# taraak/pita

Measured on AMD Instinct MI355X. Metric: walker-steps/sec (batch x T) LJ13 @ 65k walkers/GPU, higher is better.
Workload: dtype f32

## Files before the change

pita_amd/csrc/egnn_common.h:

```cpp
#pragma once
#include <cstdlib>

#include "common.h"

namespace pita {

typedef float f32x16 __attribute__((ext_vector_type(16)));
typedef float f32x4 __attribute__((ext_vector_type(4)));

constexpr int EH = 32;
constexpr int PBS = 36;
constexpr int MAT_F = 1024;
enum { M_WA = 0, M_WB, M_W2, M_WC1, M_WN1A, M_WN1B, M_WN2,
       M_WAT, M_WBT, M_W2T, M_WC1T, M_WN1AT, M_WN1BT, M_WN2T, M_COUNT };
enum { V_WRE = 0 , V_B1 = 2, V_B2, V_WATT, V_BC1, V_WC2, V_BN1,
       V_BN2, V_WRF , V_WEF , V_COUNT };
constexpr int VEC_EMB_F = 96;
constexpr int VEC_LAYER_F = V_COUNT * EH + 4;


__device__ __forceinline__ void wave_lds_fence() {
  asm volatile("s_waitcnt lgkmcnt(0)" ::: "memory");
}

// ... 82 lines not shown
      acc = __builtin_amdgcn_mfma_f32_32x32x16_bf16(as_bf16x8(w[0][st]), as_bf16x8(x[1][st]), acc, 0, 0, 0);
      acc = __builtin_amdgcn_mfma_f32_32x32x16_bf16(as_bf16x8(w[0][st]), as_bf16x8(x[0][st]), acc, 0, 0, 0);
    }
    return acc;
  }
  __device__ __forceinline__ f32x16 mul(const f32x16& in, f32x16 acc) const {
    u32x4 x[3][2];
    split(in, x);
    return mul_split(x, acc);
  }
};

constexpr float F16_SX = 1.0f, F16_SW = 16.0f;
constexpr bool F16_NODE_LAYERS = true;
constexpr float F16_UNSCALE = 1.0f / (F16_SX * F16_SW);
constexpr float DIV_ST = 32.0f;
constexpr float DIV_SV = 2048.0f;
constexpr int VEC_DIV_F = 4 * EH;
constexpr int MAT_WH = 1024;
typedef _Float16 f16x8 __attribute__((ext_vector_type(8)));
typedef _Float16 f16x2 __attribute__((ext_vector_type(2)));
__device__ __forceinline__ f16x8 as_f16x8(u32x4 v) { return __builtin_bit_cast(f16x8, v); }
__device__ __forceinline__ float f16_rem_lo(unsigned pk, float x) {
  float r;
  asm("v_fma_mix_f32 %0, %1, -1.0, %2 op_sel:[0,0,0] op_sel_hi:[1,0,0]" : "=v"(r) : "v"(pk), "v"(x));
  return r;
}
__device__ __forceinline__ float f16_rem_hi(unsigned pk, float x) {
  float r;
  asm("v_fma_mix_f32 %0, %1, -1.0, %2 op_sel:[1,0,0] op_sel_hi:[1,0,0]" : "=v"(r) : "v"(pk), "v"(x));
  return r;
}

template <>
struct WFrag<2> {
  u32x4 w[2][2];
  __device__ __forceinline__ void load(const float* __restrict__, const unsigned* __restrict__ m16, int mat, int lane) {
    const u32x4* p = reinterpret_cast<const u32x4*>(m16 + (size_t)mat * MAT_WH) + lane;
#pragma unroll
    for (int pc = 0; pc < 2; ++pc)
#pragma unroll
      for (int st = 0; st < 2; ++st) w[pc][st] = p[(pc * 2 + st) * 64];
  }
  static __device__ __forceinline__ void split(const f32x16& in, u32x4 (&x)[2][2]) {
    typedef float f32x2_t __attribute__((ext_vector_type(2)));
#pragma unroll
    for (int st = 0; st < 2; ++st)
#pragma unroll
      for (int q = 0; q < 4; ++q) {
        const float a = in[8 * st + 2 * q], b = in[8 * st + 2 * q + 1];
        const unsigned p1 = __builtin_bit_cast(unsigned, __builtin_convertvector(f32x2_t{a, b}, f16x2));
        const float ra = f16_rem_lo(p1, a), rb = f16_rem_hi(p1, b);
        x[0][st][q] = p1;
        x[1][st][q] = __builtin_bit_cast(unsigned, __builtin_convertvector(f32x2_t{ra, rb}, f16x2));
      }
  }
  __device__ __forceinline__ f32x16 mul_split(const u32x4 (&x)[2][2], f32x16 acc) const {
#pragma unroll
    for (int st = 0; st < 2; ++st) {
      acc = __builtin_amdgcn_mfma_f32_32x32x16_f16(as_f16x8(w[1][st]), as_f16x8(x[0][st]), acc, 0, 0, 0);
      acc = __builtin_amdgcn_mfma_f32_32x32x16_f16(as_f16x8(w[0][st]), as_f16x8(x[1][st]), acc, 0, 0, 0);
      acc = __builtin_amdgcn_mfma_f32_32x32x16_f16(as_f16x8(w[0][st]), as_f16x8(x[0][st]), acc, 0, 0, 0);
    }
    return acc;
  }
  __device__ __forceinline__ f32x16 mul(const f32x16& in, f32x16 acc) const {
    u32x4 x[2][2];
    split(in, x);
    return mul_split(x, acc);
  }
};

typedef float f32x2 __attribute__((ext_vector_type(2)));
constexpr float SILU_PRESCALE = -1.44269504088896341f;
__device__ __forceinline__ f32x2 silu2(f32x2 v) {
  f32x2 e;
  e.x = __builtin_amdgcn_exp2f(v.x);
  e.y = __builtin_amdgcn_exp2f(v.y);
  const f32x2 d = e + 1.0f;
  f32x2 r;
  r.x = __builtin_amdgcn_rcpf(d.x);
  r.y = __builtin_amdgcn_rcpf(d.y);
  return v * r;
}
__device__ __forceinline__ void silu16(f32x16& m) {
  f32x2 e[8];
#pragma unroll
  for (int q = 0; q < 8; ++q) {
    e[q].x = __builtin_amdgcn_exp2f(m[2 * q]);
    e[q].y = __builtin_amdgcn_exp2f(m[2 * q + 1]);
  }
#pragma unroll
  for (int q = 0; q < 8; ++q) e[q] = e[q] + 1.0f;
#pragma unroll
  for (int q = 0; q < 8; ++q) {
    e[q].x = __builtin_amdgcn_rcpf(e[q].x);
    e[q].y = __builtin_amdgcn_rcpf(e[q].y);
  }
#pragma unroll
  for (int q = 0; q < 8; ++q) {
    const f32x2 y = f32x2{m[2 * q], m[2 * q + 1]} * e[q];
    m[2 * q] = y.x;
    m[2 * q + 1] = y.y;
  }
}
__device__ __forceinline__ f32x2 silu2_scaled(f32x2 v) {
  f32x2 e;
  e.x = __builtin_amdgcn_exp2f(v.x);
  e.y = __builtin_amdgcn_exp2f(v.y);
  const f32x2 c = {1.0f / F16_SX, 1.0f / F16_SX};
  const f32x2 d = __builtin_elementwise_fma(e, c, c);
  f32x2 r;
  r.x = __builtin_amdgcn_rcpf(d.x);
  r.y = __builtin_amdgcn_rcpf(d.y);
  return v * r;
}
#ifndef PITA_SILU_BATCH
#define PITA_SILU_BATCH 8
#endif
template <bool UNSCALE>
__device__ __forceinline__ void silu16_staged(f32x16& m) {
  constexpr int Q = PITA_SILU_BATCH;
  const f32x2 c = {1.0f / F16_SX, 1.0f / F16_SX};
#pragma unroll
  for (int q0 = 0; q0 < 8; q0 += Q) {
    f32x2 v[Q], e[Q];
#pragma unroll
    for (int q = 0; q < Q; ++q) {
      v[q] = f32x2{m[2 * (q0 + q)], m[2 * (q0 + q) + 1]};
      if (UNSCALE) v[q] = v[q] * F16_UNSCALE;
    }
#pragma unroll
    for (int q = 0; q < Q; ++q) {
      e[q].x = __builtin_amdgcn_exp2f(v[q].x);
      e[q].y = __builtin_amdgcn_exp2f(v[q].y);
    }
#pragma unroll
    for (int q = 0; q < Q; ++q) e[q] = __builtin_elementwise_fma(e[q], c, c);
#pragma unroll
    for (int q = 0; q < Q; ++q) {
      e[q].x = __builtin_amdgcn_rcpf(e[q].x);
      e[q].y = __builtin_amdgcn_rcpf(e[q].y);
    }
#pragma unroll
    for (int q = 0; q < Q; ++q) {
      const f32x2 y = v[q] * e[q];
      m[2 * (q0 + q)] = y.x;
      m[2 * (q0 + q) + 1] = y.y;
    }
  }
}
__device__ __forceinline__ void silu16_out(f32x16& m) { silu16_staged<false>(m); }
__device__ __forceinline__ void silu16_acc(f32x16& m) { silu16_staged<true>(m); }

__device__ __forceinline__ float dot16(const f32x16& w, const f32x16& m) {
  f32x2 acc = {0.f, 0.f};
#pragma unroll
  for (int q = 0; q < 8; ++q)
    acc = __builtin_elementwise_fma(f32x2{w[2 * q], w[2 * q + 1]}, f32x2{m[2 * q], m[2 * q + 1]}, acc);
  return acc.x + acc.y;
}

__device__ __forceinline__ float xhalf_sum(float v) {
  const unsigned u = __float_as_uint(v);
  const auto r = __builtin_amdgcn_permlane32_swap(u, u, false, false);
  return __uint_as_float(r[0]) + __uint_as_float(r[1]);
}

__device__ __forceinline__ void frag_to_agpr(WFrag<2>& f) {
#pragma unroll
  for (int pc = 0; pc < 2; ++pc)
#pragma unroll
    for (int st = 0; st < 2; ++st) asm volatile("" : "+a"(f.w[pc][st]));
}
__device__ __forceinline__ void frag_to_agpr(WFrag<1>& f) {
#pragma unroll
  for (int pc = 0; pc < 3; ++pc)
#pragma unroll
    for (int st = 0; st < 2; ++st) asm volatile("" : "+a"(f.w[pc][st]));
}

__device__ __forceinline__ float tanh_select(float v) {
  const float a = fabsf(v);
  const float v2 = v * v;
  float p = 62.0f / 2835.0f;
  p = fmaf(p, v2, -17.0f / 315.0f);
  p = fmaf(p, v2, 2.0f / 15.0f);
  p = fmaf(p, v2, -1.0f / 3.0f);
  p = fmaf(p, v2, 1.0f);
  float small = v * p;
  const float e = __builtin_amdgcn_exp2f(2.88539008177792681f * a);
  float big = copysignf(1.0f - 2.0f * __builtin_amdgcn_rcpf(1.0f + e), v);
  asm volatile("" : "+v"(small), "+v"(big));
  return a < 0.25f ? small : big;
}

}

struct PitaDeviceGuard {
  int prev = -1;
  bool switched = false;
  explicit PitaDeviceGuard(int device) {
    if (device >= 0 && hipGetDevice(&prev) == hipSuccess && prev != device) switched = hipSetDevice(device) == hipSuccess;
  }
  ~PitaDeviceGuard() {
    if (switched) (void)hipSetDevice(prev);
  }
  PitaDeviceGuard(const PitaDeviceGuard&) = delete;
  PitaDeviceGuard& operator=(const PitaDeviceGuard&) = delete;
};

struct pita_egnn {
  pita_egnn_config cfg;
  unsigned* d_mats16 = nullptr;
  unsigned* d_mats16h = nullptr;
  float* d_mats = nullptr;
  float* d_vecs = nullptr;
  float* d_vecs_h = nullptr;
  float* d_vecs_div = nullptr;
  int* d_vjp_mark = nullptr;
  size_t vjp_mark_bytes = 0;
  const void* shape = nullptr;
  const void* shape_small = nullptr;
  int n_cu = 256;
  int device = -1;
  float* d_ws = nullptr;
  size_t ws_bytes = 0;
  float* d_divcache = nullptr;
  size_t divcache_bytes = 0;
  int* d_mark = nullptr;
  size_t mark_bytes = 0;
  int div_seq = 0;
  void* d_bk = nullptr;
  size_t bk_bytes = 0;
};
```

pita_amd/csrc/egnn_kernel.hip:

```cpp
#include "egnn_common.h"

namespace pita {

struct EgnnParams {
  const unsigned* mats16;
  const unsigned* mats16h;
  const float* mats;
  const float* vecs;
  int n_layers, in_nf, attention, tanh_on, feature_layout;
  float coord_scale;
  int mode;
  long long B;
  const float* x_in;
  const float* t;
  const float* beta;
  float* out;
  float* x;
  const float* step_tab;
  int n_steps;
  const float* noise;
  unsigned long long seed, walker_offset;
  long long step0;
  int remove_mean;
  float* drift_out;
  double* stats_out;
  int repair;
  const float* x_backup;
  int* bad_from;
};

#ifndef PITA_EGNN_RECOMPUTE_COLS
#define PITA_EGNN_RECOMPUTE_COLS 1
#endif

template <int N, int DIM, int G, int WAVES>
struct EgnnCfg {
  static constexpr int NCOL = G * N;
  static constexpr int NT = (NCOL + 31) / 32;
  static constexpr int NCOLP = NT * 32;
  static constexpr int PB_F = NCOLP * PBS;
  static constexpr int POS_F = NCOLP * DIM;
  static constexpr int WAVE_F = PB_F + 4 * POS_F;
  static __host__ __device__ constexpr int vec_f(int L) { return ((VEC_EMB_F + L * VEC_LAYER_F) + 3) & ~3; }
  static __host__ __device__ constexpr size_t lds_bytes(int L) {
    return sizeof(float) * (size_t)(vec_f(L) + WAVES * WAVE_F);
  }
};

template <int N, int DIM, int G, int WAVES, int PREC, bool SAMPLER, int OCC = 2>
__global__ void __launch_bounds__(WAVES * 64, OCC) egnn_kernel(EgnnParams p) {
  const int mode = SAMPLER ? 3 : p.mode;
  using C = EgnnCfg<N, DIM, G, WAVES>;
  constexpr int NT = C::NT;
  extern __shared__ __attribute__((aligned(16))) float lds[];

  const int L = p.n_layers;
  const int vec_f = C::vec_f(L);
  for (int i = threadIdx.x; i < VEC_EMB_F + L * VEC_LAYER_F; i += WAVES * 64) lds[i] = p.vecs[i];
  __syncthreads();

  const int wave = threadIdx.x >> 6;
  const int lane = threadIdx.x & 63;
  const int cl = lane & 31;
  const int hh = lane >> 5;
  float* PB = lds + vec_f + wave * C::WAVE_F;
  float* posbuf0 = PB + C::PB_F;
  float* posbuf1 = posbuf0 + C::POS_F;
  float* pos0 = posbuf1 + C::POS_F;
  float* xbuf = pos0 + C::POS_F;
  const float* vemb = lds;

  const long long total_waves = (long long)gridDim.x * WAVES;
  const long long quota = (p.B + total_waves - 1) / total_waves;
  const long long wbeg = ((long long)blockIdx.x * WAVES + wave) * quota;
  const long long wend = (wbeg + quota < p.B) ? wbeg + quota : p.B;
  for (long long walker0 = wbeg; walker0 < wend; walker0 += G) {
    const int nwalk = (int)((wend - walker0) < G ? (wend - walker0) : G);
    const int ncol = nwalk * N;
    const int ntile = (ncol + 31) >> 5;
    int col[NT], nodei[NT];
    bool valid[NT];
    long long wid[NT];
    float xcur[NT][DIM];
#pragma unroll
    for (int T = 0; T < NT; ++T) {
      col[T] = T * 32 + cl;
      int w = col[T] / N;
      nodei[T] = col[T] - w * N;
      wid[T] = walker0 + w;
      valid[T] = (col[T] < ncol);
      if (!valid[T]) wid[T] = p.B - 1;
      const float* src = (mode == 3 ? p.x : p.x_in);
#pragma unroll
      for (int k = 0; k < DIM; ++k) xcur[T][k] = valid[T] ? src[(walker0 * N + col[T]) * DIM + k] : 0.0f;
    }
    int bad_from[NT];
#pragma unroll
    for (int T = 0; T < NT; ++T) bad_from[T] = 0x7fffffff;
    bool mine[NT];
#pragma unroll
    for (int T = 0; T < NT; ++T) mine[T] = valid[T];
    if (PREC != 2 && p.repair) {
      bool bad = false;
      float* flag = PB;
#pragma unroll
      for (int T = 0; T < NT; ++T) {
        bool b = false;
#pragma unroll
        for (int k = 0; k < DIM; ++k) {
          const float v = (mode == 3) ? xcur[T][k] : (valid[T] ? p.out[(walker0 * N + col[T]) * DIM + k] : 0.0f);
          b = b || !__builtin_isfinite(v);
        }
        if (hh == 0) flag[col[T]] = b ? 1.0f : 0.0f;
        bad = bad || b;
      }
      if (!__any(bad)) continue;
      wave_lds_fence();
#pragma unroll
      for (int T = 0; T < NT; ++T) {
        const int cb = (col[T] < ncol) ? col[T] - nodei[T] : 0;
        float any = 0.f;
        for (int q = 0; q < N; ++q) any += flag[cb + q];
        mine[T] = valid[T] && any != 0.f;
      }
      wave_lds_fence();
      if (mode == 3) {
#pragma unroll
        for (int T = 0; T < NT; ++T) {
#pragma unroll
          for (int k = 0; k < DIM; ++k)
            xcur[T][k] = valid[T] ? p.x_backup[(walker0 * N + col[T]) * DIM + k] : 0.0f;
          if (p.stats_out && p.bad_from && valid[T]) bad_from[T] = p.bad_from[walker0 * N + col[T]];
        }
      }
    }

#pragma unroll
    for (int T = 0; T < NT; ++T)
#pragma unroll
      for (int k = 0; k < DIM; ++k)
        if (hh == 0) xbuf[col[T] * DIM + k] = xcur[T][k];
    wave_lds_fence();

    const int nsteps = (mode == 3) ? p.n_steps : 1;
    for (int step = 0; step < nsteps; ++step) {
#if PITA_EGNN_RECOMPUTE_COLS
      int col[NT], nodei[NT];
      bool valid[NT];
      long long wid[NT];
      {
        int cl_o = cl;
        asm volatile("" : "+v"(cl_o));
#pragma unroll
        for (int T = 0; T < NT; ++T) {
          col[T] = T * 32 + cl_o;
          const int w = col[T] / N;
          nodei[T] = col[T] - w * N;
          wid[T] = walker0 + w;
          valid[T] = (col[T] < ncol);
          if (!valid[T]) wid[T] = p.B - 1;
        }
      }
#endif
      float c_s[NT], c_in[NT], c_out[NT], tfeat[NT], hval[NT], bfeat[NT];
      float g2 = 0.f, gamma = 0.f, dt = 0.f, noise_scale = 0.f, sqrt_dt = 0.f;
      if (mode == 3) {
        const float* st = p.step_tab + (size_t)step * PITA_STEP_STRIDE;
        auto uni = [&](int i) {
          return __builtin_bit_cast(float, __builtin_amdgcn_readfirstlane(__builtin_bit_cast(int, st[i])));
        };
        const float u_cs = uni(PITA_ST_CS), u_cin = uni(PITA_ST_CIN), u_cout = uni(PITA_ST_COUT),
                    u_cn = uni(PITA_ST_CNOISE), u_h = uni(PITA_ST_H), u_b = uni(PITA_ST_BETA);
#pragma unroll
        for (int T = 0; T < NT; ++T) {
          c_s[T] = u_cs; c_in[T] = u_cin; c_out[T] = u_cout;
          tfeat[T] = u_cn; hval[T] = u_h; bfeat[T] = u_b;
        }
        g2 = uni(PITA_ST_G2); gamma = uni(PITA_ST_GAMMA); dt = uni(PITA_ST_DT);
        noise_scale = uni(PITA_ST_NOISE_SCALE); sqrt_dt = uni(PITA_ST_SQRT_DT);
      } else {
#pragma unroll
        for (int T = 0; T < NT; ++T) {
          float tv = p.t[wid[T]];
          bfeat[T] = p.beta ? p.beta[wid[T]] : 0.0f;
          if (mode == 0) {
            c_s[T] = 0.f; c_in[T] = 1.f; c_out[T] = 1.f; tfeat[T] = tv; hval[T] = 1.f;
          } else {
            hval[T] = tv;
            c_s[T] = 1.0f / (1.0f + tv);
            c_in[T] = 1.0f / sqrtf(1.0f + tv);
            c_out[T] = sqrtf(tv) * c_in[T];
            tfeat[T] = 0.125f * logf(tv);
          }
        }
      }

      f32x16 hfeat[NT];
#pragma unroll
      for (int T = 0; T < NT; ++T) {
#pragma unroll
        for (int k = 0; k < DIM; ++k) {
          const float xc = xbuf[col[T] * DIM + k];
          const float ps = (mode == 0) ? xc : c_in[T] * xc;
          if (hh == 0) {
            pos0[col[T] * DIM + k] = ps;
            posbuf0[col[T] * DIM + k] = ps;
          }
        }
        float a0, a1;
        if (p.in_nf == 1) {
          a0 = tfeat[T]; a1 = 0.f;
        } else if (p.feature_layout == 0) {
          a0 = (2 * nodei[T] < N) ? tfeat[T] : bfeat[T];
          a1 = (2 * nodei[T] + 1 < N) ? tfeat[T] : bfeat[T];
        } else {
          a0 = tfeat[T]; a1 = bfeat[T];
        }
        f32x16 w0 = lds_vec16(vemb + hh * 16), w1 = lds_vec16(vemb + 32 + hh * 16), eb = lds_vec16(vemb + 64 + hh * 16);
#pragma unroll
        for (int r = 0; r < 16; ++r) hfeat[T][r] = fmaf(w0[r], a0, fmaf(w1[r], a1, eb[r]));
      }
      wave_lds_fence();

      float* poscur = posbuf0;
      float* posnext = posbuf1;
      for (int l = 0; l < L; ++l) {
        const float* mats = p.mats + (size_t)l * M_COUNT * MAT_F;
        const unsigned* mats16 = p.mats16 + (size_t)l * M_COUNT * MAT_W;
        const unsigned* mats16h = p.mats16h + (size_t)l * M_COUNT * MAT_WH;
        constexpr int NPREC = (PREC == 2 && !F16_NODE_LAYERS) ? 1 : PREC;
        constexpr bool NODE16 = (PREC == 2 && F16_NODE_LAYERS);
        const unsigned* matsn = NODE16 ? mats16h : mats16;
        const float* vl = lds + VEC_EMB_F + l * VEC_LAYER_F + hh * 16;
        const bool last = (l == L - 1);
        const float aggw = last ? 0.0f : (PREC == 2 ? 1.0f / F16_SX : 1.0f);
        {
          WFrag<NPREC> wb;
          wb.load(mats, matsn, M_WB, lane);
#pragma unroll
          for (int T = 0; T < NT; ++T) {
            if (T >= ntile) continue;
            f32x16 z = {0};
            f32x16 pb = wb.mul(hfeat[T], z);
            if (NODE16) pb *= F16_UNSCALE;
            f32x4* dst = reinterpret_cast<f32x4*>(PB + col[T] * PBS + hh * 16);
            dst[0] = f32x4{pb[0], pb[1], pb[2], pb[3]};
            dst[1] = f32x4{pb[4], pb[5], pb[6], pb[7]};
            dst[2] = f32x4{pb[8], pb[9], pb[10], pb[11]};
            dst[3] = f32x4{pb[12], pb[13], pb[14], pb[15]};
          }
        }
        wave_lds_fence();

        WFrag<PREC> w2f, wc1f;
        w2f.load(mats, PREC == 2 ? mats16h : mats16, M_W2, lane);
        wc1f.load(mats, PREC == 2 ? mats16h : mats16, M_WC1, lane);
        const float a_re = lds[VEC_EMB_F + l * VEC_LAYER_F + V_WRE * EH + lane];
        const float b_att = lds[VEC_EMB_F + l * VEC_LAYER_F + V_COUNT * EH];

#pragma unroll
        for (int T = 0; T < NT; ++T) {
          if (T >= ntile) continue;
          f32x16 Ai;
          {
            WFrag<NPREC> wa;
            wa.load(mats, matsn, M_WA, lane);
            Ai = wa.mul(hfeat[T], lds_vec16(vl + V_B1 * EH));
            if (NODE16) Ai *= F16_UNSCALE;
          }
          f32x16 agg = {0};
          float xacc[DIM], pown[DIM], p0own[DIM];
#pragma unroll
          for (int k = 0; k < DIM; ++k) {
            xacc[k] = 0.f;
            pown[k] = poscur[col[T] * DIM + k];
            p0own[k] = pos0[col[T] * DIM + k];
          }
          const int cbase = col[T] - nodei[T];

          for (int dd = 1; dd < N; ++dd) {
            asm volatile("" ::: "memory");
            int j = nodei[T] + dd;
            j = (j >= N) ? j - N : j;
            const int cj = (col[T] < ncol) ? cbase + j : col[T];
            float df[DIM], radial = 0.f, ea = 0.f;
#pragma unroll
            for (int k = 0; k < DIM; ++k) {
              df[k] = pown[k] - poscur[cj * DIM + k];
              radial = fmaf(df[k], df[k], radial);
              const float e0 = p0own[k] - pos0[cj * DIM + k];
              ea = fmaf(e0, e0, ea);
            }
            f32x16 m = Ai + lds_vec16(PB + cj * PBS + hh * 16);
            m = __builtin_amdgcn_mfma_f32_32x32x2f32(a_re, hh ? ea : radial, m, 0, 0, 0);
            __builtin_amdgcn_s_setprio(0);
            if (PREC == 2) silu16_out(m); else silu16(m);
            __builtin_amdgcn_s_setprio(1);
            m = w2f.mul(m, lds_vec16(vl + V_B2 * EH));
            __builtin_amdgcn_s_setprio(0);
            if (PREC == 2) silu16_acc(m); else silu16(m);
            __builtin_amdgcn_s_setprio(1);
            if (p.attention) {
              const float att = fast_sigmoid(xhalf_sum(dot16(lds_vec16(vl + V_WATT * EH), m)) + b_att);
              m *= att;
            }
#pragma unroll
            for (int r = 0; r < 16; ++r) agg[r] = fmaf(m[r], aggw, agg[r]);
            f32x16 c1 = wc1f.mul(m, lds_vec16(vl + V_BC1 * EH));
            __builtin_amdgcn_s_setprio(0);
            if (PREC == 2) silu16_acc(c1); else silu16(c1);
            __builtin_amdgcn_s_setprio(1);
            float cs = xhalf_sum(dot16(lds_vec16(vl + V_WC2 * EH), c1));
            if (p.tanh_on) cs = accurate_tanh(cs) * p.coord_scale;
            const float inrm = __builtin_amdgcn_rcpf(__builtin_amdgcn_sqrtf(radial + 1e-8f) + 1.0f);
#pragma unroll
            for (int k = 0; k < DIM; ++k) xacc[k] = fmaf(df[k] * inrm, cs, xacc[k]);
          }
#pragma unroll
          for (int k = 0; k < DIM; ++k) {
            if (hh == 0) posnext[col[T] * DIM + k] = pown[k] + xacc[k];
          }
          if (!last) {
            WFrag<NPREC> wn;
            wn.load(mats, matsn, M_WN1A, lane);
            f32x16 n1 = wn.mul(hfeat[T], lds_vec16(vl + V_BN1 * EH));
            wn.load(mats, matsn, M_WN1B, lane);
            n1 = wn.mul(agg, n1);
            if (NODE16) silu16_acc(n1); else if (PREC == 2) silu16_out(n1); else silu16(n1);
            WFrag<PREC> wo;
            wo.load(mats, PREC == 2 ? mats16h : mats16, M_WN2, lane);
            f32x16 o = wo.mul(n1, lds_vec16(vl + V_BN2 * EH));
            if (PREC == 2) o *= F16_UNSCALE;
            hfeat[T] += o;
          }
        }
        wave_lds_fence();
        float* tmp = poscur; poscur = posnext; posnext = tmp;
      }

      float* scr = PB;
      float F[NT][DIM];
#pragma unroll
      for (int T = 0; T < NT; ++T)
#pragma unroll
        for (int k = 0; k < DIM; ++k) {
          F[T][k] = poscur[col[T] * DIM + k] - pos0[col[T] * DIM + k];
          if (hh == 0) scr[col[T] * DIM + k] = F[T][k];
        }
      wave_lds_fence();
#pragma unroll
      for (int T = 0; T < NT; ++T) {
        const int cb = (col[T] < ncol) ? col[T] - nodei[T] : 0;
#pragma unroll
        for (int k = 0; k < DIM; ++k) {
          float s = 0.f;
          for (int q = 0; q < N; ++q) s += scr[(cb + q) * DIM + k];
          F[T][k] -= s / (float)N;
        }
      }
      wave_lds_fence();

      if (mode != 3) {
#pragma unroll
        for (int T = 0; T < NT; ++T)
#pragma unroll
          for (int k = 0; k < DIM; ++k) {
            float o = F[T][k];
            if (mode >= 1) {
              const float xc = xbuf[col[T] * DIM + k];
              o = c_s[T] * xc + c_out[T] * F[T][k];
              if (mode == 2) o = (o - xc) / hval[T];
            }
            if (mine[T] && hh == 0) p.out[(walker0 * N + col[T]) * DIM + k] = o;
          }
      } else {
        float xn[NT][DIM];
        float st_d = 0.f, st_d2 = 0.f, st_n = 0.f, st_n2 = 0.f;
#pragma unroll
        for (int T = 0; T < NT; ++T) {
          float xi[4] = {0.f, 0.f, 0.f, 0.f};
          if (p.noise) {
#pragma unroll
            for (int k = 0; k < DIM; ++k)
              xi[k] = valid[T] ? p.noise[((size_t)step * p.B * N + (size_t)(walker0 * N + col[T])) * DIM + k] : 0.f;
          } else {
            philox_normal4(p.seed, p.walker_offset + (unsigned long long)wid[T], p.step0 + step, (uint32_t)nodei[T], xi);
          }
          bool take_col = true;
          if (p.stats_out && valid[T] && hh == 0) {
            if (PREC == 2) {
#pragma unroll
              for (int k = 0; k < DIM; ++k) {
                const float xc = xbuf[col[T] * DIM + k];
                const float Dth = c_s[T] * xc + c_out[T] * F[T][k];
                take_col = take_col && __builtin_isfinite(gamma * (((Dth - xc) / hval[T]) * g2));
              }
              take_col = take_col && bad_from[T] == 0x7fffffff;
              if (!take_col && bad_from[T] == 0x7fffffff) bad_from[T] = step;
            } else if (p.repair) {
              take_col = step >= bad_from[T];
            }
          }
#pragma unroll
          for (int k = 0; k < DIM; ++k) {
            const float xc = xbuf[col[T] * DIM + k];
            const float Dth = c_s[T] * xc + c_out[T] * F[T][k];
            const float sc = (Dth - xc) / hval[T];
            const float drift = gamma * (sc * g2);
            if (p.drift_out && step == nsteps - 1 && mine[T] && hh == 0)
              p.drift_out[(walker0 * N + col[T]) * DIM + k] = drift;
            const float dif = noise_scale * xi[k];
            if (p.stats_out && valid[T] && hh == 0) {
              const bool take = take_col;
              if (take) {
                st_d += drift; st_d2 = fmaf(drift, drift, st_d2);
                st_n += dif; st_n2 = fmaf(dif, dif, st_n2);
              }
            }
            xn[T][k] = xc + (drift * dt + (dif * sqrt_dt));
            if (hh == 0) scr[col[T] * DIM + k] = xn[T][k];
          }
        }
        if (p.stats_out) {
          double m4[4] = {(double)st_d, (double)st_d2, (double)st_n, (double)st_n2};
#pragma unroll
          for (int q = 0; q < 4; ++q) {
            for (int o = 32; o > 0; o >>= 1) m4[q] += __shfl_xor(m4[q], o, 64);
            if (lane == 0) atomicAdd(p.stats_out + (size_t)step * 4 + q, m4[q]);
          }
        }
        if (p.remove_mean) {
          wave_lds_fence();
#pragma unroll
          for (int T = 0; T < NT; ++T) {
            const int cb = (col[T] < ncol) ? col[T] - nodei[T] : 0;
#pragma unroll
            for (int k = 0; k < DIM; ++k) {
              float s = 0.f;
              for (int q = 0; q < N; ++q) s += scr[(cb + q) * DIM + k];
              xn[T][k] -= s / (float)N;
            }
          }
          wave_lds_fence();
        }
#pragma unroll
        for (int T = 0; T < NT; ++T)
#pragma unroll
          for (int k = 0; k < DIM; ++k)
            if (hh == 0) xbuf[col[T] * DIM + k] = xn[T][k];
        wave_lds_fence();
      }
    }

    if (mode == 3) {
#pragma unroll
      for (int T = 0; T < NT; ++T) {
#pragma unroll
        for (int k = 0; k < DIM; ++k)
          if (mine[T] && hh == 0) p.x[(walker0 * N + col[T]) * DIM + k] = xbuf[col[T] * DIM + k];
        if (PREC == 2 && p.stats_out && p.bad_from && valid[T] && hh == 0) p.bad_from[walker0 * N + col[T]] = bad_from[T];
      }
    }
    wave_lds_fence();
  }
}


struct EgnnShape {
  int n, dim, G, waves, occ;
  void (*kernel[3][2])(EgnnParams);
  size_t (*lds_bytes)(int);
};

template <int N, int DIM, int G, int WAVES>
static size_t lds_bytes_of(int L) { return EgnnCfg<N, DIM, G, WAVES>::lds_bytes(L); }

#define PITA_EGNN_SHAPE(N, DIM, G, WAVES, OCC) \
  EgnnShape { N, DIM, G, WAVES, OCC, \
              {{egnn_kernel<N, DIM, G, WAVES, 0, false, OCC>, egnn_kernel<N, DIM, G, WAVES, 0, true, OCC>}, \
               {egnn_kernel<N, DIM, G, WAVES, 1, false, OCC>, egnn_kernel<N, DIM, G, WAVES, 1, true, OCC>}, \
               {egnn_kernel<N, DIM, G, WAVES, 2, false, OCC>, egnn_kernel<N, DIM, G, WAVES, 2, true, OCC>}}, \
              lds_bytes_of<N, DIM, G, WAVES> }

static const EgnnShape kShapes[] = {
    PITA_EGNN_SHAPE(4, 2, 8, 4, 2),
    PITA_EGNN_SHAPE(13, 3, 7, 4, 2),
    PITA_EGNN_SHAPE(22, 3, 4, 4, 2),
    PITA_EGNN_SHAPE(55, 3, 1, 4, 2),
};
static const EgnnShape kShapesSmall[] = {
// ... 190 lines not shown
      }
    }
  }
  memcpy(h_vecs_h, h_vecs, sizeof(float) * VEC_EMB_F);
  pita_egnn* net = new pita_egnn();
  net->cfg = *cfg;
  net->shape = shape;
  net->shape_small = shape_small;
  hipError_t e1 = hipMalloc(&net->d_mats, n_mats * sizeof(float));
  hipError_t e2 = hipMalloc(&net->d_vecs, n_vecs * sizeof(float));
  hipError_t e0 = hipMalloc(&net->d_mats16, n_mats16 * sizeof(unsigned));
  if (e0 == hipSuccess) e0 = hipMalloc(&net->d_mats16h, n_mats16h * sizeof(unsigned));
  if (e0 == hipSuccess) e0 = hipMalloc(&net->d_vecs_h, n_vecs * sizeof(float));
  if (e0 == hipSuccess) e0 = hipMalloc(&net->d_vecs_div, (size_t)L * VEC_DIV_F * sizeof(float));
  if (e0 == hipSuccess)
    e0 = hipMemcpy(net->d_vecs_div, h_vecs_div, (size_t)L * VEC_DIV_F * sizeof(float), hipMemcpyHostToDevice);
  if (e0 == hipSuccess) e0 = hipMemcpy(net->d_mats16h, h_mats16h, n_mats16h * sizeof(unsigned), hipMemcpyHostToDevice);
  if (e0 == hipSuccess) e0 = hipMemcpy(net->d_vecs_h, h_vecs_h, n_vecs * sizeof(float), hipMemcpyHostToDevice);
  if (e1 == hipSuccess && e2 == hipSuccess && e0 == hipSuccess) {
    e1 = hipMemcpy(net->d_mats, h_mats, n_mats * sizeof(float), hipMemcpyHostToDevice);
    e2 = hipMemcpy(net->d_vecs, h_vecs, n_vecs * sizeof(float), hipMemcpyHostToDevice);
    e0 = hipMemcpy(net->d_mats16, h_mats16, n_mats16 * sizeof(unsigned), hipMemcpyHostToDevice);
  }
  if (e0 != hipSuccess && e1 == hipSuccess) e1 = e0;
  delete[] h_mats;
  delete[] h_vecs;
  delete[] h_mats16;
  delete[] h_mats16h;
  delete[] h_vecs_h;
  delete[] h_vecs_div;
  if (e1 != hipSuccess || e2 != hipSuccess) {
    (void)hipFree(net->d_mats);
    (void)hipFree(net->d_vecs);
    (void)hipFree(net->d_mats16);
    (void)hipFree(net->d_mats16h);
    (void)hipFree(net->d_vecs_h);
    (void)hipFree(net->d_vecs_div);
    delete net;
    return fail(PITA_EHIP, "pita_egnn_create: device upload failed: %s",
                hipGetErrorString(e1 != hipSuccess ? e1 : e2));
  }
  int dev = 0;
  hipDeviceProp_t prop;
  if (hipGetDevice(&dev) == hipSuccess) {
    net->device = dev;
    if (hipGetDeviceProperties(&prop, dev) == hipSuccess) net->n_cu = prop.multiProcessorCount;
  }
  size_t lds = shape->lds_bytes(L);
  hipError_t e3 = hipSuccess;
  for (int a = 0; a < 3 && e3 == hipSuccess; ++a)
    for (int b = 0; b < 2 && e3 == hipSuccess; ++b) {
      e3 = ensure_dynamic_lds(reinterpret_cast<const void*>(shape->kernel[a][b]), lds);
      if (e3 == hipSuccess && shape_small)
        e3 = ensure_dynamic_lds(reinterpret_cast<const void*>(shape_small->kernel[a][b]), shape_small->lds_bytes(L));
    }
  if (e3 != hipSuccess) {
    pita_egnn_destroy(net);
    return fail(PITA_EHIP, "pita_egnn_create: cannot reserve %zu B of LDS: %s", lds, hipGetErrorString(e3));
  }
  *out = net;
  return PITA_OK;
}

extern "C" int pita_egnn_destroy(pita_egnn_t* net) {
  if (!net) return PITA_OK;
  PitaDeviceGuard guard(net->device);
  (void)hipFree(net->d_mats);
  (void)hipFree(net->d_vecs);
  (void)hipFree(net->d_mats16);
  (void)hipFree(net->d_vjp_mark);
  (void)hipFree(net->d_mats16h);
  (void)hipFree(net->d_vecs_h);
  (void)hipFree(net->d_vecs_div);
  (void)hipFree(net->d_ws);
  (void)hipFree(net->d_bk);
  (void)hipFree(net->d_mark);
  (void)hipFree(net->d_divcache);
  delete net;
  return PITA_OK;
}

static const EgnnShape* shape_for(const pita_egnn_t* net, long long B) {
  const EgnnShape* s = static_cast<const EgnnShape*>(net->shape);
  const EgnnShape* t = static_cast<const EgnnShape*>(net->shape_small);
  if (!t) return s;
  const long long two_per_simd = (long long)net->n_cu * 8;
  const long long waves_s = (B + s->G - 1) / s->G;
  return waves_s < two_per_simd ? t : s;
}

static int egnn_launch(pita_egnn_t* net, EgnnParams& p, void* stream) {
  PitaDeviceGuard guard(net->device);
  const EgnnShape* s = shape_for(net, p.B);
  const int prec = net->cfg.precision;
  p.mats = net->d_mats;
  p.mats16 = net->d_mats16;
  p.mats16h = net->d_mats16h;
  p.vecs = prec == 2 ? net->d_vecs_h : net->d_vecs;
  p.n_layers = net->cfg.n_layers;
  p.in_nf = net->cfg.in_node_nf;
  p.attention = net->cfg.attention;
  p.tanh_on = net->cfg.tanh;
  p.feature_layout = net->cfg.feature_layout;
  p.coord_scale = net->cfg.coords_range / (float)net->cfg.n_layers;
  if (p.B == 0) return PITA_OK;
  const long long ngroups = (p.B + s->G - 1) / s->G;
  const size_t lds = s->lds_bytes(p.n_layers);
  int blocks_per_cu = (int)((160 * 1024) / lds);
  blocks_per_cu = blocks_per_cu < 1 ? 1 : (blocks_per_cu > s->occ ? s->occ : blocks_per_cu);
  long long want = (ngroups + s->waves - 1) / s->waves;
  long long cap = (long long)net->n_cu * blocks_per_cu;
  unsigned grid = (unsigned)(want < cap ? want : cap);
  if (p.mode != 3) grid = (unsigned)want;
  const int smp = p.mode == 3 ? 1 : 0;
  if (prec == 2 && smp) {
    const size_t need = sizeof(float) * (size_t)p.B * s->n * s->dim + sizeof(int) * (size_t)p.B * s->n;
    if (need > net->bk_bytes) {
      PITA_HIP_CHECK(hipStreamSynchronize((hipStream_t)stream));
      (void)hipFree(net->d_bk);
      net->d_bk = nullptr;
      net->bk_bytes = 0;
      PITA_HIP_CHECK(hipMalloc(&net->d_bk, need));
      net->bk_bytes = need;
    }
    float* xb = static_cast<float*>(net->d_bk);
    PITA_HIP_CHECK(hipMemcpyAsync(xb, p.x, sizeof(float) * (size_t)p.B * s->n * s->dim, hipMemcpyDeviceToDevice,
                                  (hipStream_t)stream));
    p.x_backup = xb;
    p.bad_from = reinterpret_cast<int*>(xb + (size_t)p.B * s->n * s->dim);
  }
  hipLaunchKernelGGL(s->kernel[prec][smp], dim3(grid), dim3(s->waves * 64), lds, (hipStream_t)stream, p);
  PITA_LAUNCH_CHECK();
  if (prec == 2) {
    p.repair = 1;
    p.vecs = net->d_vecs;
    hipLaunchKernelGGL(s->kernel[1][smp], dim3(grid), dim3(s->waves * 64), lds, (hipStream_t)stream, p);
    PITA_LAUNCH_CHECK();
  }
  return PITA_OK;
}

extern "C" int pita_egnn_sampler_work(const pita_egnn_t* net, int64_t B, double* mfma16_per_walker_step,
                                      double* mfma32_per_walker_step) {
  PITA_REQUIRE(net && B > 0 && mfma16_per_walker_step && mfma32_per_walker_step, "pita_egnn_sampler_work: bad argument");
  const EgnnShape* s = shape_for(net, B);
  const int L = net->cfg.n_layers, N = s->n, G = s->G;
  const size_t lds = s->lds_bytes(L);
  int blocks_per_cu = (int)((160 * 1024) / lds);
  blocks_per_cu = blocks_per_cu < 1 ? 1 : (blocks_per_cu > s->occ ? s->occ : blocks_per_cu);
  const long long ngroups = (B + G - 1) / G;
  long long want = (ngroups + s->waves - 1) / s->waves, cap = (long long)net->n_cu * blocks_per_cu;
  const long long total_waves = (want < cap ? want : cap) * s->waves;
  const long long quota = (B + total_waves - 1) / total_waves;
  double tiles = 0.0;
  for (long long wbeg = 0; wbeg < B; wbeg += quota) {
    const long long wend = wbeg + quota < B ? wbeg + quota : B;
    for (long long w0 = wbeg; w0 < wend; w0 += G) {
      const long long nw = (wend - w0) < G ? (wend - w0) : G;
      tiles += (double)((nw * N + 31) / 32);
    }
  }
  const double node_dense = tiles * (L * 2.0 + (L - 1) * 2.0);
  const double edge_dense = tiles * (L * 2.0 * (N - 1) + (L - 1) * 1.0);
  const double kstep = tiles * L * (N - 1);
  if (net->cfg.precision == 0) {
    *mfma16_per_walker_step = 0.0;
    *mfma32_per_walker_step = (16.0 * (node_dense + edge_dense) + kstep) / (double)B;
  } else {
    const double f16d = net->cfg.precision == 2 ? 6.0 : 12.0;
    *mfma16_per_walker_step = ((F16_NODE_LAYERS ? f16d : 12.0) * node_dense + f16d * edge_dense) / (double)B;
    *mfma32_per_walker_step = kstep / (double)B;
  }
  return PITA_OK;
}

extern "C" int pita_egnn_sampler_mapping(const pita_egnn_t* net, int64_t B, int* walkers_per_group, int64_t* waves,
                                         int64_t* wave_slots) {
  PITA_REQUIRE(net && B > 0 && walkers_per_group && waves && wave_slots, "pita_egnn_sampler_mapping: bad argument");
  const EgnnShape* s = shape_for(net, B);
  const size_t lds = s->lds_bytes(net->cfg.n_layers);
  int blocks_per_cu = (int)((160 * 1024) / lds);
  blocks_per_cu = blocks_per_cu < 1 ? 1 : (blocks_per_cu > s->occ ? s->occ : blocks_per_cu);
  const long long ngroups = (B + s->G - 1) / s->G;
  const long long want = (ngroups + s->waves - 1) / s->waves, cap = (long long)net->n_cu * blocks_per_cu;
  *walkers_per_group = s->G;
  *waves = (want < cap ? want : cap) * s->waves;
  *wave_slots = cap * s->waves;
  return PITA_OK;
}

extern "C" int pita_egnn_forward(pita_egnn_t* net, const float* t, const float* x, const float* beta, float* out,
                                 int64_t B, void* stream) {
  PITA_REQUIRE(net && t && x && out && B >= 0, "pita_egnn_forward: null argument");
  PITA_REQUIRE(beta || net->cfg.in_node_nf == 1, "pita_egnn_forward: beta required for in_node_nf=2");
  EgnnParams p{};
  p.mode = 0; p.B = B; p.x_in = x; p.t = t; p.beta = beta; p.out = out;
  return egnn_launch(net, p, stream);
}

extern "C" int pita_egnn_edm(pita_egnn_t* net, int what, const float* h, const float* x, const float* beta, float* out,
                             int64_t B, void* stream) {
  PITA_REQUIRE(net && h && x && out && B >= 0, "pita_egnn_edm: null argument");
  PITA_REQUIRE(what == 1 || what == 2, "pita_egnn_edm: what must be 1 (denoiser) or 2 (score)");
  PITA_REQUIRE(beta || net->cfg.in_node_nf == 1, "pita_egnn_edm: beta required for in_node_nf=2");
  EgnnParams p{};
  p.mode = what; p.B = B; p.x_in = x; p.t = h; p.beta = beta; p.out = out;
  return egnn_launch(net, p, stream);
}

extern "C" int pita_egnn_sampler_run(pita_egnn_t* net, float* x, int64_t B, const float* step_tab, int n_steps,
                                     const float* noise, uint64_t seed, uint64_t walker_offset, int64_t step0,
                                     int remove_mean, float* drift_out, double* stats_out, void* stream) {
  PITA_REQUIRE(net && x && step_tab && B >= 0 && n_steps >= 0, "pita_egnn_sampler_run: bad argument");
  if (n_steps == 0) return PITA_OK;
  EgnnParams p{};
  p.mode = 3; p.B = B; p.x = x; p.step_tab = step_tab; p.n_steps = n_steps; p.noise = noise;
  p.seed = seed; p.walker_offset = walker_offset; p.step0 = step0; p.remove_mean = remove_mean;
  p.drift_out = drift_out; p.stats_out = stats_out;
  return egnn_launch(net, p, stream);
}
```

Baseline: 63.60 million.

## Peel first EGNN layer using per-class embedding precompute in sampler

In the sampler path at fp16 precision, the first layer is peeled out. At that layer node features depend only on a few node classes and the relative position embedding is zero, so node projections (WB, WA, WN1A) are computed once per class and stored in LDS, and edge messages read precomputed class-pair sums. Per-tile node matmuls and the e0 distance computation are dropped for layer 0, and the layer loop is templated into first, middle and last variants. An optional f16 hi/lo split path for the edge MLP is added behind a macro that is off by default. This adds code size and register pressure, and the results depend on the class-based equivalence of the initial features.

New measurement: 64.23 million, median of 6. About the same (+1.0%).

```diff
diff --git a/pita_amd/csrc/egnn_common.h b/pita_amd/csrc/egnn_common.h
--- a/pita_amd/csrc/egnn_common.h
+++ b/pita_amd/csrc/egnn_common.h
@@ -258,6 +258,59 @@
 }
 __device__ __forceinline__ void silu16_out(f32x16& m) { silu16_staged<false>(m); }
 __device__ __forceinline__ void silu16_acc(f32x16& m) { silu16_staged<true>(m); }
+
+__device__ __forceinline__ void f16_pieces8(const float (&v)[8], const float (&r)[8], unsigned (&hi)[4], unsigned (&lo)[4]) {
+  asm("s_nop 0\n"
+      "v_fma_mixlo_f16 %0, %8, %16, 0\n"
+      "v_fma_mixhi_f16 %0, %9, %17, 0\n"
+      "v_fma_mixlo_f16 %1, %10, %18, 0\n"
+      "v_fma_mixhi_f16 %1, %11, %19, 0\n"
+      "v_fma_mixlo_f16 %2, %12, %20, 0\n"
+      "v_fma_mixhi_f16 %2, %13, %21, 0\n"
+      "v_fma_mixlo_f16 %3, %14, %22, 0\n"
+      "v_fma_mixhi_f16 %3, %15, %23, 0\n"
+      "v_fma_mixlo_f16 %4, %8, %16, -%0 op_sel_hi:[0,0,1]\n"
+      "v_fma_mixhi_f16 %4, %9, %17, -%0 op_sel:[0,0,1] op_sel_hi:[0,0,1]\n"
+      "v_fma_mixlo_f16 %5, %10, %18, -%1 op_sel_hi:[0,0,1]\n"
+      "v_fma_mixhi_f16 %5, %11, %19, -%1 op_sel:[0,0,1] op_sel_hi:[0,0,1]\n"
+      "v_fma_mixlo_f16 %6, %12, %20, -%2 op_sel_hi:[0,0,1]\n"
+      "v_fma_mixhi_f16 %6, %13, %21, -%2 op_sel:[0,0,1] op_sel_hi:[0,0,1]\n"
+      "v_fma_mixlo_f16 %7, %14, %22, -%3 op_sel_hi:[0,0,1]\n"
+      "v_fma_mixhi_f16 %7, %15, %23, -%3 op_sel:[0,0,1] op_sel_hi:[0,0,1]"
+      : "=&v"(hi[0]), "=&v"(hi[1]), "=&v"(hi[2]), "=&v"(hi[3]), "=&v"(lo[0]), "=&v"(lo[1]), "=&v"(lo[2]), "=&v"(lo[3])
+      : "v"(v[0]), "v"(v[1]), "v"(v[2]), "v"(v[3]), "v"(v[4]), "v"(v[5]), "v"(v[6]), "v"(v[7]),
+        "v"(r[0]), "v"(r[1]), "v"(r[2]), "v"(r[3]), "v"(r[4]), "v"(r[5]), "v"(r[6]), "v"(r[7]));
+}
+__device__ __forceinline__ void f16_pieces16(const f32x16& m, const f32x16& r, u32x4 (&x)[2][2]) {
+#pragma unroll
+  for (int st = 0; st < 2; ++st) {
+    float v8[8], r8[8];
+    unsigned hi[4], lo[4];
+#pragma unroll
+    for (int i = 0; i < 8; ++i) { v8[i] = m[8 * st + i]; r8[i] = r[8 * st + i]; }
+    f16_pieces8(v8, r8, hi, lo);
+#pragma unroll
+    for (int q = 0; q < 4; ++q) { x[0][st][q] = hi[q]; x[1][st][q] = lo[q]; }
+  }
+}
+__device__ __forceinline__ void silu16_split(const f32x16& m, u32x4 (&x)[2][2]) {
+  const f32x2 c = {1.0f / F16_SX, 1.0f / F16_SX};
+  f32x2 e[8];
+#pragma unroll
+  for (int q = 0; q < 8; ++q) {
+    e[q].x = __builtin_amdgcn_exp2f(m[2 * q]);
+    e[q].y = __builtin_amdgcn_exp2f(m[2 * q + 1]);
+  }
+#pragma unroll
+  for (int q = 0; q < 8; ++q) e[q] = __builtin_elementwise_fma(e[q], c, c);
+  f32x16 r;
+#pragma unroll
+  for (int q = 0; q < 8; ++q) {
+    r[2 * q] = __builtin_amdgcn_rcpf(e[q].x);
+    r[2 * q + 1] = __builtin_amdgcn_rcpf(e[q].y);
+  }
+  f16_pieces16(m, r, x);
+}
 
 __device__ __forceinline__ float dot16(const f32x16& w, const f32x16& m) {
   f32x2 acc = {0.f, 0.f};
diff --git a/pita_amd/csrc/egnn_kernel.hip b/pita_amd/csrc/egnn_kernel.hip
--- a/pita_amd/csrc/egnn_kernel.hip
+++ b/pita_amd/csrc/egnn_kernel.hip
@@ -1,3 +1,5 @@
+#include <type_traits>
+
 #include "egnn_common.h"
 
 namespace pita {
@@ -29,6 +31,10 @@
   int* bad_from;
 };
 
+#ifndef PITA_EGNN_F16_PIECES
+#define PITA_EGNN_F16_PIECES 0
+#endif
+
 #ifndef PITA_EGNN_RECOMPUTE_COLS
 #define PITA_EGNN_RECOMPUTE_COLS 1
 #endif
@@ -47,9 +53,12 @@
   }
 };
 
+enum { LK_ANY = 0, LK_FIRST, LK_MID, LK_LAST };
+
 template <int N, int DIM, int G, int WAVES, int PREC, bool SAMPLER, int OCC = 2>
 __global__ void __launch_bounds__(WAVES * 64, OCC) egnn_kernel(EgnnParams p) {
   const int mode = SAMPLER ? 3 : p.mode;
+  constexpr bool PEEL = SAMPLER && PREC == 2;
   using C = EgnnCfg<N, DIM, G, WAVES>;
   constexpr int NT = C::NT;
   extern __shared__ __attribute__((aligned(16))) float lds[];
@@ -195,6 +204,26 @@
         }
       }
 
+      const bool peel = PEEL && L >= 2;
+      auto node_class = [&](int n) {
+        return (p.in_nf == 2 && p.feature_layout == 0) ? (int)(2 * n >= N) + (int)(2 * n + 1 >= N) : 0;
+      };
+      auto embed = [&](float tf, float bf, int c, int n, bool by_class) {
+        float a0, a1;
+        if (p.in_nf == 1) {
+          a0 = tf; a1 = 0.f;
+        } else if (p.feature_layout == 0) {
+          a0 = (by_class ? c != 2 : 2 * n < N) ? tf : bf;
+          a1 = (by_class ? c == 0 : 2 * n + 1 < N) ? tf : bf;
+        } else {
+          a0 = tf; a1 = bf;
+        }
+        f32x16 w0 = lds_vec16(vemb + hh * 16), w1 = lds_vec16(vemb + 32 + hh * 16), eb = lds_vec16(vemb + 64 + hh * 16);
+        f32x16 h;
+#pragma unroll
+        for (int r = 0; r < 16; ++r) h[r] = fmaf(w0[r], a0, fmaf(w1[r], a1, eb[r]));
+        return h;
+      };
       f32x16 hfeat[NT];
 #pragma unroll
       for (int T = 0; T < NT; ++T) {
@@ -207,24 +236,20 @@
             posbuf0[col[T] * DIM + k] = ps;
           }
         }
-        float a0, a1;
-        if (p.in_nf == 1) {
-          a0 = tfeat[T]; a1 = 0.f;
-        } else if (p.feature_layout == 0) {
-          a0 = (2 * nodei[T] < N) ? tfeat[T] : bfeat[T];
-          a1 = (2 * nodei[T] + 1 < N) ? tfeat[T] : bfeat[T];
+        if (!peel) {
+          hfeat[T] = embed(tfeat[T], bfeat[T], 0, nodei[T], false);
         } else {
-          a0 = tfeat[T]; a1 = bfeat[T];
-        }
-        f32x16 w0 = lds_vec16(vemb + hh * 16), w1 = lds_vec16(vemb + 32 + hh * 16), eb = lds_vec16(vemb + 64 + hh * 16);
-#pragma unroll
-        for (int r = 0; r < 16; ++r) hfeat[T][r] = fmaf(w0[r], a0, fmaf(w1[r], a1, eb[r]));
+          hfeat[T] = f32x16{0};
+        }
       }
       wave_lds_fence();
 
       float* poscur = posbuf0;
       float* posnext = posbuf1;
-      for (int l = 0; l < L; ++l) {
+      auto layer = [&](int l, auto kind_c) __attribute__((always_inline)) {
+        constexpr int KIND = decltype(kind_c)::value;
+        constexpr bool FIRST = KIND == LK_FIRST;
+        asm volatile("" : "+s"(l));
         const float* mats = p.mats + (size_t)l * M_COUNT * MAT_F;
         const unsigned* mats16 = p.mats16 + (size_t)l * M_COUNT * MAT_W;
         const unsigned* mats16h = p.mats16h + (size_t)l * M_COUNT * MAT_WH;
@@ -232,9 +257,43 @@
         constexpr bool NODE16 = (PREC == 2 && F16_NODE_LAYERS);
         const unsigned* matsn = NODE16 ? mats16h : mats16;
         const float* vl = lds + VEC_EMB_F + l * VEC_LAYER_F + hh * 16;
-        const bool last = (l == L - 1);
+        const bool last = KIND == LK_LAST || (KIND == LK_ANY && l == L - 1);
         const float aggw = last ? 0.0f : (PREC == 2 ? 1.0f / F16_SX : 1.0f);
-        {
+        float* const ctP = PB;
+        float* const ctN = PB + 9 * PBS;
+        float* const ctH = PB + 12 * PBS;
+        float* const ctA = PB + 15 * PBS;
+        if (FIRST) {
+          const int c = cl < 3 ? cl : 2;
+          const f32x16 hc = embed(tfeat[0], bfeat[0], c, 0, true);
+          WFrag<NPREC> w;
+          w.load(mats, matsn, M_WB, lane);
+          f32x16 z = {0};
+          f32x16 pb = w.mul(hc, z);
+          if (NODE16) pb *= F16_UNSCALE;
+          w.load(mats, matsn, M_WA, lane);
+          f32x16 ai = w.mul(hc, lds_vec16(vl + V_B1 * EH));
+          if (NODE16) ai *= F16_UNSCALE;
+          w.load(mats, matsn, M_WN1A, lane);
+          const f32x16 na = w.mul(hc, lds_vec16(vl + V_BN1 * EH));
+          if (cl < 3) {
+#pragma unroll
+            for (int q = 0; q < 4; ++q) {
+              reinterpret_cast<f32x4*>(ctA + c * PBS + hh * 16)[q] = f32x4{ai[4 * q], ai[4 * q + 1], ai[4 * q + 2], ai[4 * q + 3]};
+              reinterpret_cast<f32x4*>(ctA + (3 + c) * PBS + hh * 16)[q] = f32x4{pb[4 * q], pb[4 * q + 1], pb[4 * q + 2], pb[4 * q + 3]};
+              reinterpret_cast<f32x4*>(ctN + c * PBS + hh * 16)[q] = f32x4{na[4 * q], na[4 * q + 1], na[4 * q + 2], na[4 * q + 3]};
+              reinterpret_cast<f32x4*>(ctH + c * PBS + hh * 16)[q] = f32x4{hc[4 * q], hc[4 * q + 1], hc[4 * q + 2], hc[4 * q + 3]};
+            }
+          }
+          wave_lds_fence();
+          if (cl < 9) {
+            const int ci = cl / 3, cj = cl - 3 * ci;
+            const f32x16 pr = lds_vec16(ctA + ci * PBS + hh * 16) + lds_vec16(ctA + (3 + cj) * PBS + hh * 16);
+#pragma unroll
+            for (int q = 0; q < 4; ++q)
+              reinterpret_cast<f32x4*>(ctP + cl * PBS + hh * 16)[q] = f32x4{pr[4 * q], pr[4 * q + 1], pr[4 * q + 2], pr[4 * q + 3]};
+          }
+        } else {
           WFrag<NPREC> wb;
           wb.load(mats, matsn, M_WB, lane);
 #pragma unroll
@@ -252,7 +311,7 @@
         }
         wave_lds_fence();
 
-        WFrag<PREC> w2f, wc1f;
+        std::conditional_t<KIND == LK_ANY, WFrag<PREC>, WFrag<2>> w2f, wc1f;
         w2f.load(mats, PREC == 2 ? mats16h : mats16, M_W2, lane);
         wc1f.load(mats, PREC == 2 ? mats16h : mats16, M_WC1, lane);
         const float a_re = lds[VEC_EMB_F + l * VEC_LAYER_F + V_WRE * EH + lane];
@@ -261,8 +320,9 @@
 #pragma unroll
         for (int T = 0; T < NT; ++T) {
           if (T >= ntile) continue;
+          const int ci = FIRST ? node_class(nodei[T]) : 0;
           f32x16 Ai;
-          {
+          if (!FIRST) {
             WFrag<NPREC> wa;
             wa.load(mats, matsn, M_WA, lane);
             Ai = wa.mul(hfeat[T], lds_vec16(vl + V_B1 * EH));
@@ -274,9 +334,10 @@
           for (int k = 0; k < DIM; ++k) {
             xacc[k] = 0.f;
             pown[k] = poscur[col[T] * DIM + k];
-            p0own[k] = pos0[col[T] * DIM + k];
+            p0own[k] = FIRST ? 0.f : pos0[col[T] * DIM + k];
           }
           const int cbase = col[T] - nodei[T];
+          const float* prow = ctP + ci * 3 * PBS + hh * 16;
 
           for (int dd = 1; dd < N; ++dd) {
             asm volatile("" ::: "memory");
@@ -288,25 +349,51 @@
             for (int k = 0; k < DIM; ++k) {
               df[k] = pown[k] - poscur[cj * DIM + k];
               radial = fmaf(df[k], df[k], radial);
-              const float e0 = p0own[k] - pos0[cj * DIM + k];
-              ea = fmaf(e0, e0, ea);
+              if (!FIRST) {
+                const float e0 = p0own[k] - pos0[cj * DIM + k];
+                ea = fmaf(e0, e0, ea);
+              }
             }
-            f32x16 m = Ai + lds_vec16(PB + cj * PBS + hh * 16);
-            m = __builtin_amdgcn_mfma_f32_32x32x2f32(a_re, hh ? ea : radial, m, 0, 0, 0);
+            f32x16 m = FIRST ? lds_vec16(prow + node_class(j) * PBS) : Ai + lds_vec16(PB + cj * PBS + hh * 16);
+            m = __builtin_amdgcn_mfma_f32_32x32x2f32(a_re, (hh && !FIRST) ? ea : radial, m, 0, 0, 0);
             __builtin_amdgcn_s_setprio(0);
-            if (PREC == 2) silu16_out(m); else silu16(m);
-            __builtin_amdgcn_s_setprio(1);
-            m = w2f.mul(m, lds_vec16(vl + V_B2 * EH));
+            if constexpr (KIND != LK_ANY && PITA_EGNN_F16_PIECES) {
+              u32x4 xs[2][2];
+              silu16_split(m, xs);
+              __builtin_amdgcn_s_setprio(1);
+              m = w2f.mul_split(xs, lds_vec16(vl + V_B2 * EH));
+            } else {
+              if (PREC == 2) silu16_out(m); else silu16(m);
+              __builtin_amdgcn_s_setprio(1);
+              m = w2f.mul(m, lds_vec16(vl + V_B2 * EH));
+            }
             __builtin_amdgcn_s_setprio(0);
             if (PREC == 2) silu16_acc(m); else silu16(m);
             __builtin_amdgcn_s_setprio(1);
-            if (p.attention) {
-              const float att = fast_sigmoid(xhalf_sum(dot16(lds_vec16(vl + V_WATT * EH), m)) + b_att);
-              m *= att;
+            f32x16 c1;
+            if constexpr (KIND != LK_ANY && PITA_EGNN_F16_PIECES) {
+              const float att =
+                  p.attention ? fast_sigmoid(xhalf_sum(dot16(lds_vec16(vl + V_WATT * EH), m)) + b_att) : 1.0f;
+              if (!last) {
+                const float attw = att * aggw;
+#pragma unroll
+                for (int r = 0; r < 16; ++r) agg[r] = fmaf(m[r], attw, agg[r]);
+              }
+              f32x16 attv;
+#pragma unroll
+              for (int r = 0; r < 16; ++r) attv[r] = att;
+              u32x4 xs[2][2];
+              f16_pieces16(m, attv, xs);
+              c1 = wc1f.mul_split(xs, lds_vec16(vl + V_BC1 * EH));
+            } else {
+              if (p.attention) {
+                const float att = fast_sigmoid(xhalf_sum(dot16(lds_vec16(vl + V_WATT * EH), m)) + b_att);
+                m *= att;
+              }
+#pragma unroll
+              for (int r = 0; r < 16; ++r) agg[r] = fmaf(m[r], aggw, agg[r]);
+              c1 = wc1f.mul(m, lds_vec16(vl + V_BC1 * EH));
             }
-#pragma unroll
-            for (int r = 0; r < 16; ++r) agg[r] = fmaf(m[r], aggw, agg[r]);
-            f32x16 c1 = wc1f.mul(m, lds_vec16(vl + V_BC1 * EH));
             __builtin_amdgcn_s_setprio(0);
             if (PREC == 2) silu16_acc(c1); else silu16(c1);
             __builtin_amdgcn_s_setprio(1);
@@ -322,8 +409,13 @@
           }
           if (!last) {
             WFrag<NPREC> wn;
-            wn.load(mats, matsn, M_WN1A, lane);
-            f32x16 n1 = wn.mul(hfeat[T], lds_vec16(vl + V_BN1 * EH));
+            f32x16 n1;
+            if (FIRST) {
+              n1 = lds_vec16(ctN + ci * PBS + hh * 16);
+            } else {
+              wn.load(mats, matsn, M_WN1A, lane);
+              n1 = wn.mul(hfeat[T], lds_vec16(vl + V_BN1 * EH));
+            }
             wn.load(mats, matsn, M_WN1B, lane);
             n1 = wn.mul(agg, n1);
             if (NODE16) silu16_acc(n1); else if (PREC == 2) silu16_out(n1); else silu16(n1);
@@ -331,11 +423,25 @@
             wo.load(mats, PREC == 2 ? mats16h : mats16, M_WN2, lane);
             f32x16 o = wo.mul(n1, lds_vec16(vl + V_BN2 * EH));
             if (PREC == 2) o *= F16_UNSCALE;
-            hfeat[T] += o;
+            if (FIRST) hfeat[T] = lds_vec16(ctH + ci * PBS + hh * 16) + o;
+            else hfeat[T] += o;
           }
         }
         wave_lds_fence();
         float* tmp = poscur; poscur = posnext; posnext = tmp;
+      };
+      if constexpr (PEEL) {
+        if (peel) {
+          layer(0, std::integral_constant<int, LK_FIRST>{});
+          for (int l = 1; l < L - 1; ++l) layer(l, std::integral_constant<int, LK_MID>{});
+          layer(L - 1, std::integral_constant<int, LK_LAST>{});
+        } else {
+#ifndef EXP_NOFALLBACK
+          for (int l = 0; l < L; ++l) layer(l, std::integral_constant<int, LK_ANY>{});
+#endif
+        }
+      } else {
+        for (int l = 0; l < L; ++l) layer(l, std::integral_constant<int, LK_ANY>{});
       }
 
       float* scr = PB;
@@ -832,15 +938,18 @@
   long long want = (ngroups + s->waves - 1) / s->waves, cap = (long long)net->n_cu * blocks_per_cu;
   const long long total_waves = (want < cap ? want : cap) * s->waves;
   const long long quota = (B + total_waves - 1) / total_waves;
-  double tiles = 0.0;
+  double tiles = 0.0, groups = 0.0;
   for (long long wbeg = 0; wbeg < B; wbeg += quota) {
     const long long wend = wbeg + quota < B ? wbeg + quota : B;
     for (long long w0 = wbeg; w0 < wend; w0 += G) {
       const long long nw = (wend - w0) < G ? (wend - w0) : G;
       tiles += (double)((nw * N + 31) / 32);
+      groups += 1.0;
     }
   }
-  const double node_dense = tiles * (L * 2.0 + (L - 1) * 2.0);
+  const bool peel = net->cfg.precision == 2 && L >= 2;
+  const double node_dense = peel ? tiles * ((L - 1) * 2.0 + (L - 1) * 2.0 - 1.0) + groups * 3.0
+                                 : tiles * (L * 2.0 + (L - 1) * 2.0);
   const double edge_dense = tiles * (L * 2.0 * (N - 1) + (L - 1) * 1.0);
   const double kstep = tiles * L * (N - 1);
   if (net->cfg.precision == 0) {
```
